# salesforce/gorp

Measured on AMD Instinct MI355X. Metric: lines/sec (Gorp.extract: product-DFA match + capture offsets; results as narrow rows (int8 id + uint8 offsets, 9 B/line)), higher is better.
Workload: dtype u8

## Files before the change

gorp_amd/csrc/gx_kernels.hip:

```cpp
#include "gx_rows.hpp"
#include "gx_hop_dev.hpp"

namespace gx {

namespace {

constexpr int GENERIC_MAX_REGS = 96;

template <typename CH>
__device__ __forceinline__ int class_of(const GxDev& T, CH ch) {
    uint32_t c = static_cast<uint32_t>(ch);
    if (sizeof(CH) == 1 || c < 256u) return T.cls256[c];
    int lo = 0, hi = T.n_hi;
    while (hi - lo > 1) {
        int mid = (lo + hi) >> 1;
        if (T.hi_lo[mid] <= c) lo = mid; else hi = mid;
    }
    return T.hi_cls[lo];
}

template <typename CH>
__device__ bool pike_capture(const GxDev& T, int k, const CH* __restrict__ s, int64_t len, int32_t* __restrict__ scratch, int32_t* __restrict__ caps_out) {
    const uint32_t base = T.pike_off[k], n_inst = T.pike_off[k + 1] - base;
    const uint32_t* code = T.pike_code + 2ull * base;
// ... 389 lines not shown
            const uint4 w0 = make_uint4(wv.x, wv.y, wv.z, wv.w);
            const bool full0 = rel + 16u <= len;
            const uint32_t bx = outside_bits(w0.x, lo4, k4), by = outside_bits(w0.y, lo4, k4);
            const uint32_t bz = outside_bits(w0.z, lo4, k4), bw = outside_bits(w0.w, lo4, k4);
            const bool ok0 = full0 & (((or3(bx, by, bz) | bw) & HI_BITS) == 0u);
            bool step = act && !ok0;
            uint32_t mask = 0xFFFFu;
            if (step && !full0) {
                mask = window_mask(0u, len, rel);
                step = !partial_window_ok(bx, by, bz, bw, mask);
            }
            const bool masked = __any(step && !full0);
            if (step) {
                if (want_caps) {
                    if (L.simple_ops) {
                        if (!masked) row = steps16<TIER, true, false, true>(w0, mask, W, row, rel, regs);
                        else row = steps16<TIER, true, true, true>(w0, mask, W, row, rel, regs);
                    } else {
                        if (!masked) row = steps16<TIER, true, false, false>(w0, mask, W, row, rel, regs);
                        else row = steps16<TIER, true, true, false>(w0, mask, W, row, rel, regs);
                    }
                } else {
                    if (!masked) row = steps16<TIER, false, false, false>(w0, mask, W, row, rel, regs);
                    else row = steps16<TIER, false, true, false>(w0, mask, W, row, rel, regs);
                }
                const uint32_t acc = state_acc<TIER>(W, row);
                lo4 = splat_byte0(acc);
                k4 = splat_byte1(acc);
            }
            more = more && row != dead_row;
        }
        if (walking) pos += SLICE_BYTES;
        __builtin_amdgcn_fence(__ATOMIC_RELEASE, "wavefront");
        __builtin_amdgcn_wave_barrier();
    }
}

template <typename OFF, int TIER>
hipError_t launch_slices_t(const GxDev& dev, const GxLds& lds, const uint8_t* lds_image, const uint8_t* at_global, dim3 grid, dim3 block,
                           const GxBatch& b, hipStream_t stream) {
    hipError_t e = allow_full_lds(&k_extract_slices<OFF, TIER>);
    if (e != hipSuccess) return e;
    hipLaunchKernelGGL((k_extract_slices<OFF, TIER>), grid, block, lds.total_bytes, stream, dev, lds, lds_image, at_global,
                       static_cast<const uint8_t*>(b.data), static_cast<const OFF*>(b.offsets), b.n, row_out(dev, b), b.match_only, b.strip_eol);
    return hipGetLastError();
}

#ifndef GX_HOP_LEAVE
#define GX_HOP_LEAVE 24u
#endif
#ifndef GX_HOP_SERVICE
#define GX_HOP_SERVICE 64u
#endif
constexpr uint64_t HOP_POOL_CHUNK = 64;
constexpr uint32_t HOP_SLICE = GX_HOP_SLICE_BYTES, HOP_SLICE_ROW = GX_HOP_SLICE_BYTES + 16u, HOP_SLICE_KEEP = 24;

typedef __attribute__((address_space(1))) const UnalignedWindow GlobalWindow;
template <bool WIDE, bool GUARDED>
__device__ __forceinline__ u32x4 load_chunk16(const uint8_t* src, const uint8_t* data_end, uint32_t units, uint32_t& high) {
    u32x4 a = {0u, 0u, 0u, 0u}, b2 = {0u, 0u, 0u, 0u};
    if (!GUARDED) {
        a = reinterpret_cast<GlobalWindow*>(reinterpret_cast<uintptr_t>(src))->v;
        if (WIDE) b2 = reinterpret_cast<GlobalWindow*>(reinterpret_cast<uintptr_t>(src + 16))->v;
    } else {
        uint32_t w[8] = {0, 0, 0, 0, 0, 0, 0, 0};
#pragma nounroll
        for (int q = 0; q < (WIDE ? 32 : 16); ++q)
            if (src + q < data_end) w[q >> 2] |= static_cast<uint32_t>(src[q]) << ((q & 3) * 8);
        a = u32x4{w[0], w[1], w[2], w[3]}; b2 = u32x4{w[4], w[5], w[6], w[7]};
    }
    if (!WIDE) return a;
    const uint32_t hi[8] = {a.x, a.y, a.z, a.w, b2.x, b2.y, b2.z, b2.w};
    uint32_t acc = 0u;
#pragma unroll
    for (uint32_t q = 0; q < 8u; ++q) {
        uint32_t m = 0xFF00FF00u;
        if (2u * q + 1u >= units) m = 2u * q >= units ? 0u : 0x0000FF00u;
        acc |= hi[q] & m;
    }
    high |= acc;
    return u32x4{__builtin_amdgcn_perm(a.y, a.x, 0x06040200u), __builtin_amdgcn_perm(a.w, a.z, 0x06040200u),
                 __builtin_amdgcn_perm(b2.y, b2.x, 0x06040200u), __builtin_amdgcn_perm(b2.w, b2.z, 0x06040200u)};
}
__device__ __forceinline__ bool chunk_in_run(const u32x4& v, uint32_t runinfo) {
    const uint32_t lo4 = splat_byte0(runinfo), k4 = splat_byte1(runinfo);
    const uint32_t f = (v.x | (v.x - lo4) | (v.x + k4)) | (v.y | (v.y - lo4) | (v.y + k4)) | (v.z | (v.z - lo4) | (v.z + k4)) | (v.w | (v.w - lo4) | (v.w + k4));
    return (f & HI_BITS) == 0u;
}
#ifndef GX_HOP_SPEC
#define GX_HOP_SPEC 1
#endif
#ifndef GX_HOP_SPEC_UNITS
#define GX_HOP_SPEC_UNITS 24
#endif
#ifndef GX_HOP_SPEC_BATCH
#define GX_HOP_SPEC_BATCH 8u
#endif
#ifndef GX_HOP_SPEC_MIN
#define GX_HOP_SPEC_MIN 0u
#endif


template <typename OFF, bool WIDE>
__global__ void __launch_bounds__(768) __attribute__((amdgpu_waves_per_eu(1, 3)))
k_extract_hop_slices(GxDev T, GxLds L, const uint8_t* __restrict__ lds_image, const uint8_t* __restrict__ at_global,
                     const uint8_t* __restrict__ data, const OFF* __restrict__ off, uint64_t n, RowOut out, int match_only, int strip_eol,
                     uint32_t* __restrict__ oversize_flag, uint32_t seq, unsigned long long* __restrict__ stamps,
                     uint32_t* __restrict__ pool_ctr, uint32_t pool_base, uint64_t n_static,
                     uint8_t* __restrict__ wide_flags, uint32_t* __restrict__ wide_any) {
    {
        extern __shared__ __attribute__((aligned(16))) uint8_t gx_smem[];
        const uint4* src = reinterpret_cast<const uint4*>(lds_image);
        uint4* dst = reinterpret_cast<uint4*>(gx_smem);
        for (uint32_t c = threadIdx.x; c < L.table_bytes / 16; c += blockDim.x) dst[c] = src[c];
    }
    __syncthreads();
#ifdef GX_DEV
    unsigned long long ph[6] = {0, 0, 0, 0, 0, 0}, ph_t = __builtin_amdgcn_s_memtime();
    unsigned long long dv[6] = {0, 0, 0, 0, 0, 0};
    const unsigned long long hs_begin = __builtin_amdgcn_s_memrealtime();
#define HS_STAMP(slot) do { const unsigned long long now_ = __builtin_amdgcn_s_memtime(); ph[slot] += now_ - ph_t; ph_t = now_; } while (0)
#else
#define HS_STAMP(slot) do { } while (0)
#endif
    HopTab H;
    H.rows = at_global;
    H.hops = at_global + L.c_base;
    H.row_bytes = L.row_bytes;
    H.info_off = L.ncls * 4u;
    H.n_hot = L.rec_indexed;
    H.lrow_cols = (2u * L.ncls + 3u) & ~3u;
    H.sets = L.hop_sets;
    const uint32_t lane = threadIdx.x & 63u;
    const uint32_t wave = threadIdx.x >> 6;
    const uint32_t slice = L.stage + wave * L.stage_bytes;
    const uint32_t regs = L.regs + wave * L.regs_wave_bytes + 128u + lane * 2u;
    const uint8_t* data_end = data + (static_cast<uint64_t>(off[n]) << (WIDE ? 1 : 0));
    const uint32_t row0 = match_only ? L.m_start : L.u_start, dead_row = match_only ? L.m_dead : L.u_dead;
    const uint8_t* fin_g = L.at != 0u ? nullptr : at_global + L.fin_tags;
    const uint32_t fin_lds = L.at;

    const uint64_t nwaves = static_cast<uint64_t>(gridDim.x) * L.nwaves;
    const uint64_t per_wave = (n_static + nwaves - 1) / nwaves;
    const uint64_t wid = static_cast<uint64_t>(blockIdx.x) * L.nwaves + wave;
    const uint64_t range_lo = min(n_static, wid * per_wave);
    uint64_t range_hi = min(n_static, range_lo + per_wave);
    uint64_t next = range_lo;
    const uint64_t pool_chunks = (n - n_static + HOP_POOL_CHUNK - 1) / HOP_POOL_CHUNK;
    bool pool_done = pool_ctr == nullptr;

    bool has_line = false;
    uint64_t i = 0, o0 = 0;
    uint32_t len = 0, pos = 0, row = row0;
    const uint32_t my = slice + lane * HOP_SLICE_ROW;
    bool line_wide = false;
    const uint64_t total_units = static_cast<uint64_t>(off[n]);
    uint64_t win_base = ~0ull;
    OFF w_lo = 0, w_hi = 0;
    auto refill = [&](uint64_t base) {
        win_base = base;
        const uint64_t a = min(base + lane, n);
        w_lo = off[a];
        w_hi = off[min(a + 1u, n)];
    };
    refill(range_lo);
    FinAhead F;
    bool fin_here = false;
    uint32_t near_end = 0u;
    HopKept K;
    const bool all_hot = L.rec_indexed >= L.sort_chunk;

    for (;;) {
        const bool finished = has_line && (pos >= len || row == dead_row);
        const uint32_t idle = static_cast<uint32_t>(__popcll(__ballot(finished || !has_line)));
        const bool service = idle >= GX_HOP_SERVICE || !__any(has_line && !finished);
        if (service && finished) {
            const bool rows_here = !(WIDE && line_wide);
            if (!match_only) lds_st<uint16_t>(regs - 128u, static_cast<uint16_t>(len));
            if (!match_only && L.fin_state_off != 0u) {
                const uint8_t* recp = at_global + L.fin_state_off + static_cast<uint64_t>(row) * L.fin_state_rec;
                if (!fin_here) F.load(recp, T.max_groups);
                if (rows_here) store_row<TIER_HOP>(out, i, 0, F.at(recp), regs, len, T.max_groups, L.fin_unset);
                fin_here = false;
            } else {
                const int32_t hot_info = static_cast<int16_t>(lds_ld<uint16_t>(L.acc_tab + 2u * min(row, H.n_hot - 1u)));
                int32_t info = hot_info >= 0 && !match_only ? hot_info * 16 : hot_info;
                if (row >= H.n_hot) info = *reinterpret_cast<const int32_t*>(H.rows + (static_cast<uint64_t>(row) * H.row_bytes + H.info_off));
                if (match_only) out.id(i, info);
                else if (rows_here) store_row<TIER_HOP>(out, i, info, fin_rec<TIER_HOP>(info, fin_lds, fin_g), regs, len, T.max_groups, L.fin_unset);
            }
            if (WIDE) {
                wide_flags[i] = line_wide ? 1 : 0;
                if (line_wide) __hip_atomic_store(wide_any, seq, __ATOMIC_RELAXED, __HIP_MEMORY_SCOPE_AGENT);
            }
            has_line = false;
        }
#ifdef GX_DEV
        if (service) ++dv[3];
#endif
        HS_STAMP(5);
        if (service && next >= range_hi && !pool_done) {
            uint32_t t = 0u;
            if (lane == 0u) t = __hip_atomic_fetch_add(pool_ctr, 1u, __ATOMIC_RELAXED, __HIP_MEMORY_SCOPE_AGENT) - pool_base;
            t = static_cast<uint32_t>(__builtin_amdgcn_readfirstlane(static_cast<int>(t)));
            if (t < pool_chunks) {
                next = n_static + static_cast<uint64_t>(t) * HOP_POOL_CHUNK;
                range_hi = min(n, next + HOP_POOL_CHUNK);
            } else pool_done = true;
        }
        const uint64_t free_mask = __ballot(!has_line);
        if (service && free_mask && next < range_hi) {
            const uint32_t rank = static_cast<uint32_t>(__popcll(free_mask & ((1ull << lane) - 1ull)));
            const uint64_t cand = next + rank;
            const uint32_t n_free = static_cast<uint32_t>(__popcll(free_mask));
            const bool in_win = next >= win_base && next - win_base + n_free <= 64u;
            OFF o_lo = 0, o_hi = 0;
            if (in_win) {
                const int src = static_cast<int>(static_cast<uint32_t>(next - win_base) + rank) & 63;
                o_lo = __shfl(w_lo, src);
                o_hi = __shfl(w_hi, src);
            }
            if (!has_line && cand < range_hi) {
                i = cand;
                if (!in_win) { o_lo = off[i]; o_hi = off[i + 1]; }
                o0 = o_lo;
                int64_t len64 = static_cast<int64_t>(static_cast<uint64_t>(o_hi) - o0);
                if (strip_eol) len64 = WIDE ? trim_eol(reinterpret_cast<const uint16_t*>(data) + o0, len64) : trim_eol(data + o0, len64);
                line_wide = false;
                if (WIDE && len64 > 65535) wide_flags[i] = 0;
                if (len64 > 65535) {
                    announce_left_line(oversize_flag, seq);
                } else {
                    has_line = true;
                    len = static_cast<uint32_t>(len64);
                    pos = 0;
                    row = row0;
                    near_end = static_cast<uint64_t>(o_hi) + 16u > total_units ? 0x10000u : 0u;
                }
            }
            next = min(range_hi, next + static_cast<uint64_t>(n_free));
            refill(next);
// ... 157 lines not shown
                    }
                }
                __builtin_amdgcn_fence(__ATOMIC_RELEASE, "wavefront");
                __builtin_amdgcn_wave_barrier();
                __builtin_amdgcn_fence(__ATOMIC_ACQUIRE, "wavefront");
                uint32_t got = 0u;
                bool alive = longrun;
                for (uint32_t k = 0; __builtin_amdgcn_ballot_w64(alive && k < units) != 0ull; ++k) {
                    const bool look = alive && k < units;
                    const uint32_t bits = look ? lds_ld<uint8_t>(BITS + first + k) : 0xFFu;
                    if (look) {
                        got += 16u * static_cast<uint32_t>(__builtin_ctz(~bits | 0x100u));
                        alive = bits == 0xFFu;
                    }
                }
                extra = min(got, rest0);
            }
        }
        pos += extra;
        if (!match_only && L.fin_state_off != 0u) {
            if (has_line && !fin_here && (pos >= len || row == dead_row)) {
                F.load(at_global + L.fin_state_off + static_cast<uint64_t>(row) * L.fin_state_rec, T.max_groups);
                fin_here = true;
            }
        }
        __builtin_amdgcn_fence(__ATOMIC_RELEASE, "wavefront");
        __builtin_amdgcn_wave_barrier();
        HS_STAMP(2);
#ifdef GX_DEV
        ++ph[4];
#endif
    }
#ifdef GX_DEV
    if (stamps && lane == 0) {
        unsigned long long* st = stamps + 16ull * (static_cast<uint64_t>(blockIdx.x) * L.nwaves + wave);
        for (int q = 0; q < 6; ++q) st[q] = ph[q];
        st[6] = hs_begin;
        st[7] = __builtin_amdgcn_s_memrealtime();
        for (int q = 0; q < 4; ++q) st[8 + q] = dv[q];
        st[12] = K.dev_iters;
        st[13] = K.dev_lane_iters;
    }
#endif
}

}

namespace {
uint64_t hop_slices_blocks(uint64_t n, uint32_t nwaves, int num_cus) {
    uint64_t blocks = static_cast<uint64_t>(num_cus);
    const uint64_t need = (n + 256ull * nwaves - 1) / (256ull * nwaves);
    return blocks > need ? need : blocks;
}
uint64_t hop_slices_static(uint64_t n) { return n - (n / 4) / HOP_POOL_CHUNK * HOP_POOL_CHUNK; }
}

uint32_t hop_slices_tickets(uint64_t n, uint32_t nwaves, int num_cus) {
    if (n == 0) return 0u;
    const uint64_t chunks = (n - hop_slices_static(n) + HOP_POOL_CHUNK - 1) / HOP_POOL_CHUNK;
    return static_cast<uint32_t>(chunks + hop_slices_blocks(n, nwaves, num_cus) * nwaves);
}

hipError_t launch_extract_hop_slices(const GxDev& dev, const GxLds& lds, const uint8_t* lds_image, const uint8_t* at_global, int num_cus,
                                     const GxBatch& b, hipStream_t stream, unsigned long long* stamps) {
    if (b.n == 0) return hipSuccess;
    const uint64_t blocks = hop_slices_blocks(b.n, lds.nwaves, num_cus);
    const uint64_t n_static = b.chunk_ctr ? hop_slices_static(b.n) : b.n;
    const dim3 grid(static_cast<unsigned>(blocks)), block(lds.nwaves * 64);
    auto go = [&](auto kernel, auto offsets) -> hipError_t {
        hipError_t e = allow_full_lds(kernel);
        if (e != hipSuccess) return e;
        hipLaunchKernelGGL(kernel, grid, block, lds.total_bytes, stream, dev, lds, lds_image, at_global, static_cast<const uint8_t*>(b.data), offsets, b.n, row_out(dev, b),
                           (b.match_only != 0 || !dev.has_capture) ? 1 : 0, b.strip_eol, b.oversize_flag, b.seq, stamps, b.chunk_ctr, b.chunk_base, n_static,
                           b.wide_flags, b.wide_any);
        return hipGetLastError();
    };
    if (b.wide) {
        if (!b.wide_flags || !b.wide_any) return hipErrorInvalidValue;
        if (b.offsets64) return go(&k_extract_hop_slices<uint64_t, true>, static_cast<const uint64_t*>(b.offsets));
        return go(&k_extract_hop_slices<uint32_t, true>, static_cast<const uint32_t*>(b.offsets));
    }
    if (b.offsets64) return go(&k_extract_hop_slices<uint64_t, false>, static_cast<const uint64_t*>(b.offsets));
    return go(&k_extract_hop_slices<uint32_t, false>, static_cast<const uint32_t*>(b.offsets));
}

hipError_t launch_narrow_units(const GxBatch& b, uint8_t* bytes_at_first_unit, uint8_t* flags, hipStream_t stream) {
    if (b.n == 0) return hipSuccess;
    hipError_t e = hipMemsetAsync(flags, 0, b.n, stream);
    if (e != hipSuccess) return e;
    const dim3 grid(256u * 16u), block(256);
    if (b.offsets64) hipLaunchKernelGGL((k_narrow_units<uint64_t>), grid, block, 0, stream, static_cast<const uint16_t*>(b.data), static_cast<const uint64_t*>(b.offsets), b.n, bytes_at_first_unit, flags);
    else hipLaunchKernelGGL((k_narrow_units<uint32_t>), grid, block, 0, stream, static_cast<const uint16_t*>(b.data), static_cast<const uint32_t*>(b.offsets), b.n, bytes_at_first_unit, flags);
    return hipGetLastError();
}
hipError_t launch_extract_flagged(const GxDev& dev, const GxBatch& b, const uint8_t* flags, hipStream_t stream, const uint32_t* any_word) {
    if (b.n == 0) return hipSuccess;
    const dim3 grid(dev.pike_off ? dev.pike_blocks : 256u * 4u), block(256);
    const uint16_t* units = static_cast<const uint16_t*>(b.data);
#define GX_FLAGGED(OFF, MS, NEXT) hipLaunchKernelGGL((k_extract_flagged<OFF, MS>), grid, block, 0, stream, dev, units, static_cast<const OFF*>(b.offsets), b.n, flags, row_out(dev, b), b.match_only, NEXT, b.strip_eol, any_word, b.seq)
    if (b.offsets64) { if (dev.m_next16) GX_FLAGGED(uint64_t, uint16_t, dev.m_next16); else GX_FLAGGED(uint64_t, uint32_t, dev.m_next32); }
    else { if (dev.m_next16) GX_FLAGGED(uint32_t, uint16_t, dev.m_next16); else GX_FLAGGED(uint32_t, uint32_t, dev.m_next32); }
#undef GX_FLAGGED
    return hipGetLastError();
}
hipError_t launch_extract_listed(const GxDev& dev, const GxBatch& b, const uint64_t* list, uint64_t count, hipStream_t stream) {
    if (count == 0) return hipSuccess;
    if (!b.wide || !b.offsets64) return hipErrorInvalidValue;
// ... 61 lines not shown
```

gorp_amd/csrc/gx_lanes.hip:

```cpp
#include "gx_rows.hpp"

namespace gx {

namespace {

struct LanesIO {
    const uint8_t* image;
    const uint8_t* at_global;
    const uint8_t* data;
    const void* off;
    uint64_t n;
    RowOut rows;
    uint32_t* oversize_flag;
    uint32_t seq;
    int32_t max_groups;
    int32_t strip_eol;
    uint32_t chunk_lines;
    uint32_t sort_lds;
    uint32_t* chunk_ctr;
    uint32_t chunk_base;
#ifdef GX_DEV
    unsigned long long* stamps;
#endif
};
// ... 121 lines not shown
            bool more = valid && !oversize && len > 0u;
            auto line_chunk = [&](uint32_t at_byte, bool wanted) -> u32x4 {
                u32x4 v = {0u, 0u, 0u, 0u};
                if (wanted && at_byte < len) {
                    const uint8_t* src = line + at_byte;
                    if (src + 16 <= data_end) v = reinterpret_cast<const UnalignedWindow*>(src)->v;
                    else {
                        uint32_t w[4] = {0, 0, 0, 0};
                        for (int b = 0; b < 16; ++b)
                            if (src + b < data_end) w[b >> 2] |= static_cast<uint32_t>(src[b]) << ((b & 3) * 8);
                        v = u32x4{w[0], w[1], w[2], w[3]};
                    }
                }
                return v;
            };
            for (uint32_t seg = 0; __any(more); seg += KCH * 16u) {
                u32x4 pre[KCH];
    #pragma unroll
                for (int k = 0; k < KCH; ++k) pre[k] = line_chunk(seg + 16u * k, more);
    #pragma unroll 1
                for (int k = 0; k < KCH; ++k) {
                    const uint32_t rel = seg + 16u * k;
                    const bool act = more && rel < len;
                    if (!__any(act)) break;
                    const uint4 w0 = make_uint4(pre[0].x, pre[0].y, pre[0].z, pre[0].w);
    #pragma unroll
                    for (int q = 0; q + 1 < KCH; ++q) pre[q] = pre[q + 1];
                    const bool full0 = rel + 16u <= len;
                    const uint32_t bx = outside_bits(w0.x, lo4, k4), by = outside_bits(w0.y, lo4, k4);
                    const uint32_t bz = outside_bits(w0.z, lo4, k4), bw = outside_bits(w0.w, lo4, k4);
                    const bool ok0 = full0 & (((or3(bx, by, bz) | bw) & HI_BITS) == 0u);
                    bool step = act && !ok0;
                    uint32_t mask = 0xFFFFu;
                    if (step && !full0) {
                        mask = window_mask(0u, len, rel);
                        step = !partial_window_ok(bx, by, bz, bw, mask);
                    }
                    const bool masked = __any(step && !full0);
                    if (step) {
                        if (!masked) row = steps16<TIER, CAPTURE, false, SIMPLE>(w0, mask, W, row, rel, regs);
                        else row = steps16<TIER, CAPTURE, true, SIMPLE>(w0, mask, W, row, rel, regs);
                        acc = state_acc<TIER>(W, row);
                        lo4 = splat_byte0(acc);
                        k4 = splat_byte1(acc);
                    }
                    more = more && row != dead_row && rel + 16u < len;
                }
            }

            const int32_t info = state_info<TIER>(W, row);
            if (!CAPTURE) {
                if (valid && !oversize) io.rows.match_id[i] = info;
            } else {
                auto result = [&](auto emit) { return line_result<TIER>(info, L.fin_tags, fin_g, regs, len, G, emit); };
                const bool full_tile = contiguous && __all(valid) && !__any(oversize);
                const uint32_t area_bytes = L.regs_wave_bytes - L.stage_bytes;
                if (!PACKED) store_tile<ROWS_DENSE, false>(io.rows, slots, i, lane, valid && !oversize, false, out_area, area_bytes, len, result);
                else if (io.rows.format == ROWS_U8) store_tile<ROWS_U8, true>(io.rows, slots, i, lane, valid && !oversize, full_tile, out_area, area_bytes, len, result);
                else store_tile<ROWS_U16, false>(io.rows, slots, i, lane, valid && !oversize, full_tile, out_area, area_bytes, len, result);
            }
            __builtin_amdgcn_fence(__ATOMIC_ACQ_REL, "wavefront");
            __builtin_amdgcn_wave_barrier();
            if (!SORTED) j = next_ticket();
        }
        if (!SORTED) break;
        __syncthreads();
    }
#ifdef GX_DEV
    if (io.stamps && threadIdx.x == 0) {
        io.stamps[2 * blockIdx.x] = __builtin_amdgcn_s_memtime() - dev_t0;
        io.stamps[2 * blockIdx.x + 1] = __builtin_amdgcn_s_memrealtime() - dev_r0;
    }
#endif
}

template <typename OFF, int TIER, bool CAPTURE, bool SIMPLE, bool PACKED, bool SORTED>
hipError_t launch_lanes_s(const GxLds& lds, const LanesIO& io, dim3 grid, hipStream_t stream) {
    constexpr int KCH = 13;
    hipError_t e = allow_full_lds(&k_extract_lanes<OFF, KCH, TIER, CAPTURE, SIMPLE, PACKED, SORTED>);
    if (e != hipSuccess) return e;
    hipLaunchKernelGGL((k_extract_lanes<OFF, KCH, TIER, CAPTURE, SIMPLE, PACKED, SORTED>), grid, dim3(lds.nwaves * 64), lds.total_bytes, stream, lds, io);
    return hipGetLastError();
}
template <typename OFF, int TIER, bool CAPTURE, bool SIMPLE, bool PACKED>
hipError_t launch_lanes_t(const GxLds& lds, const LanesIO& io, dim3 grid, hipStream_t stream) {
    if (io.chunk_lines) return launch_lanes_s<OFF, TIER, CAPTURE, SIMPLE, PACKED, true>(lds, io, grid, stream);
    return launch_lanes_s<OFF, TIER, CAPTURE, SIMPLE, PACKED, false>(lds, io, grid, stream);
}
template <typename OFF, int TIER>
hipError_t launch_lanes_m(bool capture, bool simple, bool packed, const GxLds& lds, const LanesIO& io, dim3 grid, hipStream_t stream) {
    if (!capture) return launch_lanes_t<OFF, TIER, false, false, false>(lds, io, grid, stream);
    if (simple) return packed ? launch_lanes_t<OFF, TIER, true, true, true>(lds, io, grid, stream) : launch_lanes_t<OFF, TIER, true, true, false>(lds, io, grid, stream);
    return packed ? launch_lanes_t<OFF, TIER, true, false, true>(lds, io, grid, stream) : launch_lanes_t<OFF, TIER, true, false, false>(lds, io, grid, stream);
}

}

uint32_t lanes_sorted_tickets(uint64_t n, uint32_t chunk_lines, int num_cus) {
    const uint64_t nchunks = (n + chunk_lines - 1) / chunk_lines;
    return static_cast<uint32_t>(nchunks + (static_cast<uint64_t>(num_cus) < nchunks ? static_cast<uint64_t>(num_cus) : nchunks));
}

hipError_t launch_extract_lanes(const GxDev& dev, const GxLds& lds, const uint8_t* lds_image, const uint8_t* at_global, int num_cus,
                                const GxBatch& b, hipStream_t stream, unsigned long long* dev_stamps) {
    if (b.n == 0) return hipSuccess;
    const uint64_t tiles = (b.n + 63) >> 6;
    uint64_t blocks = static_cast<uint64_t>(num_cus);
// ... 47 lines not shown
```

gorp_amd/csrc/gx_rows.hpp:

```cpp
#pragma once
#include "gx_walk.hpp"

namespace gx {

struct RowOut {
    int32_t* match_id;
    int32_t* caps;
    uint8_t* rows;
    unsigned long long* overflow;
    RowFormat format;
    uint32_t slots;

    __device__ __forceinline__ void id(uint64_t i, int32_t k) const {
        if (format == ROWS_U8) rows[i * row_bytes(ROWS_U8, slots)] = static_cast<uint8_t>(encode_id(ROWS_U8, k));
        else if (format == ROWS_U16) *reinterpret_cast<uint16_t*>(rows + i * row_bytes(ROWS_U16, slots)) = static_cast<uint16_t>(encode_id(ROWS_U16, k));
        else match_id[i] = k;
    }
    __device__ __forceinline__ void cap(uint64_t i, int t, int32_t v) const {
        if (format == ROWS_DENSE) { caps[i * static_cast<uint64_t>(slots) + t] = v; return; }
        const RowUnit u = encode_offset(format, v);
        if (u.clipped && overflow) atomicAdd(overflow, 1ull);
        uint8_t* p = rows + i * row_bytes(format, slots) + row_unit_bytes(format) * (1u + t);
        if (format == ROWS_U8) *p = static_cast<uint8_t>(u.unit);
        else *reinterpret_cast<uint16_t*>(p) = static_cast<uint16_t>(u.unit);
// ... 29 lines not shown
    }
}
template <int TIER>
__device__ __forceinline__ void resolve_tags(const u32x4& t, uint32_t regs, uint32_t len, uint32_t hop_unset, int32_t (&pb)[4], int32_t (&pe)[4]) {
    uint32_t tw[4], vb[4], ve[4];
    tag_columns<TIER>(t, regs, tw, vb, ve);
#pragma unroll
    for (int q = 0; q < 4; ++q) tag_offsets<TIER>(tw[q], vb[q], ve[q], len, hop_unset, pb[q], pe[q]);
}

struct FinRec {
    uint32_t fin_lds;
    const uint8_t* fin_g;
    uint32_t rec;
    bool global;
    __device__ __forceinline__ u32x4 tags(int g0) const {
        return global ? *reinterpret_cast<const u32x4*>(fin_g + rec + 4u * g0) : lds_ld<u32x4>(fin_lds + rec + 4u * g0);
    }
    __device__ __forceinline__ uint32_t id_of(int G) const {
        const uint32_t id_at = rec + 16u * static_cast<uint32_t>((G + 3) >> 2);
        return global ? *reinterpret_cast<const uint16_t*>(fin_g + id_at) : lds_ld<uint16_t>(fin_lds + id_at);
    }
};
template <int TIER>
__device__ __forceinline__ FinRec fin_rec(int32_t info, uint32_t fin_lds, const uint8_t* fin_g) {
    const bool global = TIER == TIER_L2 || TIER == TIER_RECG || (TIER == TIER_HOP && fin_g != nullptr);
    return FinRec{fin_lds, fin_g, info >= 0 ? static_cast<uint32_t>(info) : 0u, global};
}

struct FinAhead {
    u32x4 t0 = {0u, 0u, 0u, 0u}, t1 = {0u, 0u, 0u, 0u}, t2 = {0u, 0u, 0u, 0u};
    uint32_t id = 0u;
    __device__ __forceinline__ void load(const uint8_t* __restrict__ recp, int G) {
        const int nblk = (G + 3) >> 2;
        t0 = *reinterpret_cast<const u32x4*>(recp);
        t1 = *reinterpret_cast<const u32x4*>(recp + (nblk > 1 ? 16 : 0));
        t2 = *reinterpret_cast<const u32x4*>(recp + (nblk > 2 ? 32 : 0));
        id = *reinterpret_cast<const uint16_t*>(recp + 16 * nblk);
    }
    struct At {
        u32x4 t0, t1, t2;
        uint32_t id;
        const uint8_t* recp;
        __device__ __forceinline__ u32x4 tags(int g0) const {
            if (g0 >= 12) return *reinterpret_cast<const u32x4*>(recp + 4 * g0);
            const u32x4 a = t0, b = t1, c = t2;
            return g0 == 0 ? a : g0 == 4 ? b : c;
        }
        __device__ __forceinline__ uint32_t id_of(int) const { return id; }
    };
    __device__ __forceinline__ At at(const uint8_t* recp) const { return At{t0, t1, t2, id, recp}; }
};

template <int TIER, typename EMIT>
__device__ __forceinline__ int32_t line_result(int32_t info, uint32_t fin_lds, const uint8_t* fin_g, uint32_t regs, uint32_t len, int G,
                                               EMIT emit, uint32_t hop_unset = 0u) {
    const uint32_t rec = info >= 0 ? static_cast<uint32_t>(info) : 0u;
    const uint32_t id_at = rec + 16u * static_cast<uint32_t>((G + 3) >> 2);
    uint32_t id;
    const bool FIN_GLOBAL = TIER == TIER_L2 || TIER == TIER_RECG || (TIER == TIER_HOP && fin_g != nullptr);
    if (FIN_GLOBAL) id = *reinterpret_cast<const uint16_t*>(fin_g + id_at);
    else id = lds_ld<uint16_t>(fin_lds + id_at);
    for (int g0 = 0; g0 < G; g0 += 4) {
        u32x4 t;
        if (FIN_GLOBAL) t = *reinterpret_cast<const u32x4*>(fin_g + rec + 4u * g0);
        else t = lds_ld<u32x4>(fin_lds + rec + 4u * g0);
        uint32_t tw[4], vb[4], ve[4];
        tag_columns<TIER>(t, regs, tw, vb, ve);
#pragma unroll
        for (int q = 0; q < 4; ++q) {
            if (g0 + q < G) {
                int32_t pb, pe;
                tag_offsets<TIER>(tw[q], vb[q], ve[q], len, hop_unset, pb, pe);
                emit(g0 + q, pb, pe);
            }
        }
    }
    return info >= 0 ? static_cast<int32_t>(static_cast<int16_t>(id)) : info;
}

struct __attribute__((packed)) UnalignedU32x4 { u32x4 v; };
struct __attribute__((packed)) UnalignedU32x2 { u32x2 v; };
struct __attribute__((packed)) UnalignedU32 { uint32_t v; };
struct __attribute__((packed)) UnalignedU16 { uint16_t v; };

template <int TIER, typename REC>
__device__ __forceinline__ void store_row(const RowOut& out, uint64_t i, int32_t info, const REC& rec, uint32_t regs, uint32_t len, int G,
                                          uint32_t hop_unset = 0u) {
    const RowFormat f = out.format;
    const int32_t mid = info >= 0 ? static_cast<int32_t>(static_cast<int16_t>(rec.id_of(G))) : info;
    uint8_t* row = f != ROWS_DENSE ? out.rows + i * row_bytes(f, out.slots) : reinterpret_cast<uint8_t*>(out.caps + i * static_cast<uint64_t>(out.slots));
    if (f == ROWS_DENSE) out.match_id[i] = mid;
    uint32_t carry = encode_id(f, mid);
    uint32_t clipped = 0u;
    const bool may_clip = __builtin_amdgcn_ballot_w64(len > static_cast<uint32_t>(row_max_offset(f))) != 0ull;
    for (int g0 = 0; g0 < G; g0 += 4) {
        int32_t pb[4], pe[4];
        resolve_tags<TIER>(rec.tags(g0), regs, len, hop_unset, pb, pe);
        const int cnt = G - g0 < 4 ? G - g0 : 4;
        if (f == ROWS_DENSE) {
            uint8_t* dst = row + 8u * g0;
            if (cnt == 4) {
                reinterpret_cast<UnalignedU32x4*>(dst)->v = u32x4{static_cast<uint32_t>(pb[0]), static_cast<uint32_t>(pe[0]), static_cast<uint32_t>(pb[1]), static_cast<uint32_t>(pe[1])};
                reinterpret_cast<UnalignedU32x4*>(dst + 16)->v = u32x4{static_cast<uint32_t>(pb[2]), static_cast<uint32_t>(pe[2]), static_cast<uint32_t>(pb[3]), static_cast<uint32_t>(pe[3])};
            } else {
#pragma unroll
                for (int q = 0; q < 4; ++q) if (q < cnt) reinterpret_cast<UnalignedU32x2*>(dst + 8 * q)->v = u32x2{static_cast<uint32_t>(pb[q]), static_cast<uint32_t>(pe[q])};
            }
            continue;
        }
        uint32_t hb[4], he[4];
        if (!may_clip) {
#pragma unroll
            for (int q = 0; q < 4; ++q) { hb[q] = static_cast<uint32_t>(pb[q]) & row_unset(f); he[q] = static_cast<uint32_t>(pe[q]) & row_unset(f); }
        } else {
#pragma unroll
            for (int q = 0; q < 4; ++q) {
                const RowUnit b = encode_offset(f, pb[q]), e = encode_offset(f, pe[q]);
                hb[q] = b.unit;
                he[q] = e.unit;
                clipped += b.clipped + e.clipped;
            }
        }
        if (f == ROWS_U16) {
            uint8_t* dst = row + 4u * g0;
            if (cnt == 4) {
                reinterpret_cast<UnalignedU32x4*>(dst)->v = u32x4{carry | hb[0] << 16, he[0] | hb[1] << 16, he[1] | hb[2] << 16, he[2] | hb[3] << 16};
                carry = he[3];
            } else {
#pragma unroll
                for (int q = 0; q < 4; ++q) {
                    if (q >= cnt) break;
                    reinterpret_cast<UnalignedU32*>(dst + 4 * q)->v = carry | hb[q] << 16;
                    carry = he[q];
                }
            }
        } else {
            uint8_t* dst = row + 2u * g0;
            if (cnt == 4) {
                reinterpret_cast<UnalignedU32x2*>(dst)->v = u32x2{carry | hb[0] << 8 | he[0] << 16 | hb[1] << 24, he[1] | hb[2] << 8 | he[2] << 16 | hb[3] << 24};
                carry = he[3];
            } else {
#pragma unroll
                for (int q = 0; q < 4; ++q) {
                    if (q >= cnt) break;
                    reinterpret_cast<UnalignedU16*>(dst + 2 * q)->v = static_cast<uint16_t>(carry | hb[q] << 8);
                    carry = he[q];
                }
            }
        }
    }
    if (f != ROWS_DENSE) {
        if (f == ROWS_U8) row[2 * G] = static_cast<uint8_t>(carry);
        else reinterpret_cast<UnalignedU16*>(row + 4 * G)->v = static_cast<uint16_t>(carry);
        if (clipped && out.overflow) atomicAdd(out.overflow, static_cast<unsigned long long>(clipped));
    }
}

template <RowFormat F, bool CLIP, typename RESULT>
__device__ __forceinline__ void store_tile(const RowOut& out, uint32_t slots, uint64_t i, uint32_t lane, bool valid, bool full, uint32_t area,
                                           uint32_t area_bytes, uint32_t len, RESULT result, uint32_t dev_flags = 0u) {
    (void)dev_flags;
    if (F != ROWS_DENSE) {
        constexpr uint32_t U = row_unit_bytes(F);
        const uint32_t row_b = row_bytes(F, slots);
        constexpr int32_t max = row_max_offset(F);
        auto st = [&](uint32_t lds_at, int32_t v) {
            if (U == 1) lds_st<uint8_t>(lds_at, static_cast<uint8_t>(v));
            else lds_st<uint16_t>(lds_at, static_cast<uint16_t>(v));
        };
        const bool rows_aligned = (reinterpret_cast<uintptr_t>(out.rows) & 15u) == 0u;
        uint32_t clipped = 0;
        if (full && rows_aligned && 64u * row_b + 16u <= area_bytes) {
            const uint32_t my_row = area + lane * row_b;
            int32_t id;
            if (!CLIP || !__any(len > static_cast<uint32_t>(max))) {
                id = result([&](int g, int32_t pb, int32_t pe) {
                    st(my_row + U + 2u * U * g, pb);
                    st(my_row + 2u * U + 2u * U * g, pe);
                });
            } else {
                id = result([&](int g, int32_t pb, int32_t pe) {
                    clipped += (pb > max ? 1u : 0u) + (pe > max ? 1u : 0u);
                    st(my_row + U + 2u * U * g, pb > max ? max : pb);
                    st(my_row + 2u * U + 2u * U * g, pe > max ? max : pe);
                });
            }
            st(my_row, id);
            __builtin_amdgcn_fence(__ATOMIC_ACQ_REL, "wavefront");
            __builtin_amdgcn_wave_barrier();
            uint8_t* out_rows = out.rows + (i - lane) * static_cast<uint64_t>(row_b);
            for (uint32_t c = lane; c < 4u * row_b; c += 64u) {
#ifdef GX_DEV
                if (dev_flags & 2u) { __builtin_nontemporal_store(lds_ld<u32x4>(area + (c << 4)), reinterpret_cast<u32x4*>(out_rows + (c << 4))); continue; }
                if ((dev_flags & 4u) && c != 0u) continue;
#endif
                *reinterpret_cast<u32x4*>(out_rows + (c << 4)) = lds_ld<u32x4>(area + (c << 4));
            }
        } else if (valid) {
            using Unit = typename std::conditional<U == 1, uint8_t, uint16_t>::type;
            Unit* rp = reinterpret_cast<Unit*>(out.rows) + i * static_cast<uint64_t>(1u + slots);
            auto gst = [&](uint32_t k, int32_t v) { rp[k] = static_cast<Unit>(v); };
            const int32_t id = result([&](int g, int32_t pb, int32_t pe) {
                if (CLIP) {
                    clipped += (pb > max ? 1u : 0u) + (pe > max ? 1u : 0u);
                    gst(1 + 2 * g, pb > max ? max : pb);
                    gst(2 + 2 * g, pe > max ? max : pe);
                } else {
                    gst(1 + 2 * g, pb);
                    gst(2 + 2 * g, pe);
                }
            });
            gst(0, id);
        }
        if (CLIP && out.overflow && __any(clipped != 0u)) {
            uint32_t sum = clipped;
#pragma unroll
            for (int d = 32; d >= 1; d >>= 1) sum += static_cast<uint32_t>(__shfl_xor(static_cast<int>(sum), d));
            if (lane == 0) atomicAdd(out.overflow, static_cast<unsigned long long>(sum));
        }
    } else {
        const uint32_t row_b = slots * 4u;
        const bool caps_aligned = ((reinterpret_cast<uintptr_t>(out.caps) | reinterpret_cast<uintptr_t>(out.match_id)) & 15u) == 0u;
        if (full && caps_aligned && 64u * row_b + 256u <= area_bytes) {
            const uint32_t my_row = area + lane * row_b;
            const int32_t id = result([&](int g, int32_t pb, int32_t pe) {
                lds_st<u32x2>(my_row + 8u * g, u32x2{static_cast<uint32_t>(pb), static_cast<uint32_t>(pe)});
            });
            const uint32_t ids = area + 64u * row_b;
            lds_st<uint32_t>(ids + 4u * lane, static_cast<uint32_t>(id));
            __builtin_amdgcn_fence(__ATOMIC_ACQ_REL, "wavefront");
            __builtin_amdgcn_wave_barrier();
            uint8_t* dst = reinterpret_cast<uint8_t*>(out.caps + (i - lane) * static_cast<uint64_t>(slots));
            for (uint32_t c = lane; c < 4u * row_b; c += 64u)
                *reinterpret_cast<u32x4*>(dst + (c << 4)) = lds_ld<u32x4>(area + (c << 4));
            if (lane < 16u)
                *reinterpret_cast<u32x4*>(out.match_id + (i - lane) + 4u * lane) = lds_ld<u32x4>(ids + 16u * lane);
        } else if (valid) {
            int32_t* cp = out.caps + i * static_cast<uint64_t>(slots);
            out.match_id[i] = result([&](int g, int32_t pb, int32_t pe) {
                cp[2 * g] = pb;
                cp[2 * g + 1] = pe;
            });
        }
    }
}

}
```

gorp_amd/csrc/gx_service.hip:

```cpp
#include "gx_tile_body.hpp"

namespace gx {

namespace {

__device__ __forceinline__ uint32_t sys_load(const uint32_t* p) { return __hip_atomic_load(p, __ATOMIC_RELAXED, __HIP_MEMORY_SCOPE_SYSTEM); }

template <int MODE>
__global__ void __launch_bounds__(64)
k_one_service(GxLds L, const uint8_t* __restrict__ image, const uint32_t* __restrict__ mailbox, int32_t* __restrict__ answer, uint32_t* __restrict__ state,
              uint32_t last, int max_groups, unsigned long long idle_ticks, unsigned long long life_ticks) {
    {
        extern __shared__ __attribute__((aligned(16))) uint8_t gx_smem[];
        const uint4* src = reinterpret_cast<const uint4*>(image);
        uint4* dst = reinterpret_cast<uint4*>(gx_smem);
        for (uint32_t c = threadIdx.x; c < L.table_bytes / 16; c += blockDim.x) dst[c] = src[c];
    }
    __syncthreads();
    const uint32_t lane = threadIdx.x;
    WalkTab W;
    W.at = nullptr;
    W.row_bytes = L.row_bytes;
    W.ops_off = L.ops_off;
    W.ops = L.ops;
    W.acc_tab = L.acc_tab;
    W.ncls = L.ncls;
    W.indexed = L.rec_indexed;
    const uint32_t stage = L.stage;
    const uint32_t regs = L.regs + 128u + lane * 2u;
    const int G = max_groups;
    const unsigned long long born = __builtin_amdgcn_s_memrealtime();
    unsigned long long idle_since = born;
    bool announced = false;
    for (;;) {
        uint32_t w = lane < 16u ? sys_load(mailbox + lane) : 0u;
        const uint32_t seq = static_cast<uint32_t>(__builtin_amdgcn_readlane(static_cast<int>(w), 0));
        const uint32_t head = static_cast<uint32_t>(__builtin_amdgcn_readlane(static_cast<int>(w), 1));
        if (seq != last) {
            const uint32_t len = head & 0xFFFFu;
            if (announced) { if (lane == 0) __hip_atomic_store(state, 1u, __ATOMIC_RELAXED, __HIP_MEMORY_SCOPE_SYSTEM); announced = false; }
            if (lane >= 2u && lane < 16u) lds_st<uint32_t>(stage + 4u * (lane - 2u), w);
            if (len > 56u) {
                const uint32_t lines = (len - 56u + 59u) / 60u;
                for (uint32_t c0 = 0; c0 < lines; c0 += 4u) {
                    const uint32_t cl = c0 + (lane >> 4), d = lane & 15u;
                    const bool mine = cl < lines;
                    for (;;) {
                        const uint32_t v = mine ? sys_load(mailbox + 16u * (1u + cl) + d) : seq;
                        const bool tag_ok = d != 0u || v == seq;
                        if (__builtin_amdgcn_ballot_w64(!tag_ok) == 0ull) {
                            if (mine && d != 0u) lds_st<uint32_t>(stage + 56u + 60u * cl + 4u * (d - 1u), v);
                            break;
                        }
                        __builtin_amdgcn_s_sleep(2);
                    }
                }
            }
            __builtin_amdgcn_fence(__ATOMIC_RELEASE, "wavefront");
            __builtin_amdgcn_wave_barrier();
            __builtin_amdgcn_fence(__ATOMIC_ACQUIRE, "wavefront");
            const bool on = lane == 0u;
            const uint32_t out = stage + L.stage_bytes - 272u;
            int32_t result;
            if (MODE == 0) {
                const uint32_t mrow = walk<TIER_LDS, false, false>(W, stage, 0u, false, L.m_start, 0u, on ? len : 0u, on, L.m_dead, regs);
                result = state_info<TIER_LDS>(W, mrow);
                if (on) lds_st<uint32_t>(out, static_cast<uint32_t>(result));
            } else {
                const uint32_t urow = walk<TIER_LDS, true, true>(W, stage, 0u, false, L.u_start, 0u, on ? len : 0u, on, L.u_dead, regs);
                const int32_t info = state_info<TIER_LDS>(W, urow);
                result = line_result<TIER_LDS>(info, L.fin_tags, nullptr, regs, len, G, [&](int g, int32_t pb, int32_t pe) {
                    if (on) lds_st<u32x2>(out + 4u + 8u * g, u32x2{static_cast<uint32_t>(pb), static_cast<uint32_t>(pe)});
                });
                if (on) lds_st<uint32_t>(out, static_cast<uint32_t>(result));
            }
            __builtin_amdgcn_fence(__ATOMIC_RELEASE, "wavefront");
            __builtin_amdgcn_wave_barrier();
            __builtin_amdgcn_fence(__ATOMIC_ACQUIRE, "wavefront");
            if (lane < 1u + 2u * static_cast<uint32_t>(MODE == 0 ? 0 : G)) answer[lane] = static_cast<int32_t>(lds_ld<uint32_t>(out + 4u * lane));
            __builtin_amdgcn_fence(__ATOMIC_RELEASE, "");
            if (on) __hip_atomic_store(reinterpret_cast<uint32_t*>(answer) + 1 + 2 * max_groups, seq, __ATOMIC_RELEASE, __HIP_MEMORY_SCOPE_SYSTEM);
            last = seq;
            idle_since = __builtin_amdgcn_s_memrealtime();
            if (idle_since - born > life_ticks) {
                if (lane == 0) __hip_atomic_store(state, 2u, __ATOMIC_RELEASE, __HIP_MEMORY_SCOPE_SYSTEM);
                announced = true;
                continue;
            }
            continue;
        }
        if (announced) break;
        const unsigned long long now = __builtin_amdgcn_s_memrealtime();
        if ((head >> 16) & 1u || now - idle_since > idle_ticks || now - born > life_ticks) {
            if (lane == 0) __hip_atomic_store(state, 2u, __ATOMIC_RELEASE, __HIP_MEMORY_SCOPE_SYSTEM);
            __builtin_amdgcn_fence(__ATOMIC_SEQ_CST, "");
            announced = true;
            continue;
        }
        __builtin_amdgcn_s_sleep(1);
    }
}

}

hipError_t launch_one_service(int mode, const GxLds& lds, const uint8_t* lds_image, const uint32_t* mailbox, int32_t* answer, uint32_t* state,
                              uint32_t last_seq, int max_groups, unsigned long long idle_ticks, unsigned long long life_ticks, hipStream_t stream) {
    if (mode == 0) {
        hipError_t e = allow_full_lds(&k_one_service<0>);
        if (e != hipSuccess) return e;
        hipLaunchKernelGGL((k_one_service<0>), dim3(1), dim3(64), lds.total_bytes, stream, lds, lds_image, mailbox, answer, state, last_seq, max_groups, idle_ticks, life_ticks);
    } else {
        hipError_t e = allow_full_lds(&k_one_service<1>);
        if (e != hipSuccess) return e;
        hipLaunchKernelGGL((k_one_service<1>), dim3(1), dim3(64), lds.total_bytes, stream, lds, lds_image, mailbox, answer, state, last_seq, max_groups, idle_ticks, life_ticks);
    }
    return hipGetLastError();
}

}
```

gorp_amd/csrc/gx_tile_body.hpp:

```cpp
#pragma once
#include "gx_rows.hpp"
#include "gx_hop_dev.hpp"

namespace gx {

namespace {

struct TileIO {
    const uint8_t* image;
    const uint8_t* at_global;
    const uint8_t* data;
    const void* off;
    uint64_t n;
    RowOut rows;
    uint32_t* oversize_flag;
    uint32_t seq;
    int32_t max_groups;
    int32_t strip_eol;
    uint32_t* steal;
    uint32_t steal_parity;
    uint32_t share64;
    uint8_t* wide_flags;
    uint32_t* wide_any;
    int32_t* state_out;
// ... 401 lines not shown
        if (io.strip_eol && cur.mode != 2) {
            if (end > start && lds_ld<uint8_t>(stage + end - 1u) == 0x0Au) --end;
            if (end > start && lds_ld<uint8_t>(stage + end - 1u) == 0x0Du) --end;
        }
        if (cur.mode == 2) {
            if (lane == cur.a) announce_left_line(io.oversize_flag, io.seq);
        } else if (MODE == 0 && HOP) {
            const uint32_t mrow = walk_hop<false>(H, L.rec_indexed >= L.sort_chunk, stage, L.m_start, start, end, true, L.m_dead, regs, hop_second);
            int32_t first = static_cast<int16_t>(lds_ld<uint16_t>(L.acc_tab + 2u * min(mrow, H.n_hot - 1u)));
            if (wave_any(mrow >= H.n_hot)) {
                if (mrow >= H.n_hot) first = *reinterpret_cast<const int32_t*>(H.rows + (static_cast<uint64_t>(mrow) * H.row_bytes + H.info_off));
            }
            if (valid) io.rows.match_id[i] = first;
            GX_STAMP(2);
        } else if (MODE == 0) {
            const uint32_t mrow = walk<TIER, false, false>(Wm, stage, bitmap, use_map, L.m_start, start, end, true, L.m_dead, regs);
            if (valid) io.rows.match_id[i] = state_info<TIER>(Wm, mrow);
            if ((TIER == TIER_LDS || TIER == TIER_L2) && io.state_out && valid)
                io.state_out[i] = mrow == L.m_dead ? -1 : static_cast<int32_t>(TIER == TIER_LDS ? (mrow - L.m_start) / L.row_bytes : mrow - L.m_start);
            GX_STAMP(2);
        } else {
            int32_t info;
            if (HOP) {
                const uint32_t urow = walk_hop<true>(H, L.rec_indexed >= L.sort_chunk, stage, L.u_start, start, end, true, L.u_dead, regs, hop_second);
                const int32_t hot_info = static_cast<int16_t>(lds_ld<uint16_t>(L.acc_tab + 2u * min(urow, H.n_hot - 1u)));
                info = hot_info >= 0 ? hot_info * 16 : hot_info;
                if (wave_any(urow >= H.n_hot)) {
                    if (urow >= H.n_hot) info = *reinterpret_cast<const int32_t*>(H.rows + (static_cast<uint64_t>(urow) * H.row_bytes + H.info_off));
                }
            } else if (MODE == 1 || L.u_start != 0xFFFFFFFFu) {
                uint32_t urow;
                if (MODE == 1 || L.simple_ops) urow = walk<TIER, true, true>(Wc, stage, bitmap, use_map, L.u_start, start, end, true, L.u_dead, regs);
                else urow = walk<TIER, true, false>(Wc, stage, bitmap, use_map, L.u_start, start, end, true, L.u_dead, regs);
                info = state_info<TIER>(Wc, urow);
            } else {
                const uint32_t mrow = walk<TIER, false, false>(Wm, stage, bitmap, use_map, L.m_start, start, end, true, L.m_dead, regs);
                const int32_t k = state_info<TIER>(Wm, mrow);
                info = k;
                uint32_t crow = GT ? 0u : L.m_dead;
                if (k >= 0) crow = lds_ld<uint32_t>(L.c_rule + 8u * k);
                if (L.simple_ops) crow = walk<TIER, true, true>(Wc, stage, bitmap, use_map, crow, start, end, k >= 0, 0xFFFFFFFFu, regs);
                else crow = walk<TIER, true, false>(Wc, stage, bitmap, use_map, crow, start, end, k >= 0, 0xFFFFFFFFu, regs);
                if (k >= 0) {
                    info = state_info<TIER>(Wc, crow);
                    if (info < 0) info = -2 - k;
                }
            }
            GX_STAMP(2);
            if (WIDE && wide_line) info = -1;
            const uint32_t len = end - start;
            if (HOP) lds_st<uint16_t>(regs - 128u, static_cast<uint16_t>(len));
            const uint8_t* fin_g = GT && !(HOP && L.at != 0u) ? io.at_global + L.fin_tags : nullptr;
            const uint32_t fin_lds = HOP ? L.at : L.fin_tags;
            auto result = [&](auto emit) { return line_result<TIER>(info, fin_lds, fin_g, regs, len, G, emit, L.fin_unset); };
            const bool full_tile = cur.a == 0u && cur.b == 64u;
#ifdef GX_DEV
            const uint32_t dev_flags = io.dev_flags;
#else
            const uint32_t dev_flags = 0u;
#endif
            constexpr RowFormat FMT = PACKED == 2 ? ROWS_U8 : PACKED == 1 ? ROWS_U16 : ROWS_DENSE;
            store_tile<FMT, FMT == ROWS_U8>(io.rows, slots, i, lane, valid, full_tile, stage, L.stage_bytes, len, result, dev_flags);
        }
        if (WIDE) {
            if (valid || (cur.mode == 2 && lane == cur.a)) io.wide_flags[i] = (wide_line && cur.mode != 2) ? 1 : 0;
            if (__builtin_amdgcn_ballot_w64(wide_line && valid && cur.mode != 2) != 0ull && lane == 0)
                __hip_atomic_store(io.wide_any, io.seq, __ATOMIC_RELAXED, __HIP_MEMORY_SCOPE_AGENT);
        }
        __builtin_amdgcn_fence(__ATOMIC_ACQ_REL, "wavefront");
        __builtin_amdgcn_wave_barrier();
        GX_STAMP(3);
#ifdef GX_DEV
        ++dev_tiles;
#endif
        if (!has_next) break;
        if (!same_group) {
            t1 = t2;
            need_t2 = true;
        }
        cur = nxt;
        tile = ntile;
        no0 = nno0;
        no1 = nno1;
    }
#ifdef GX_DEV
    if (io.stamps && lane == 0) {
        unsigned long long* s = io.stamps + 8ull * (static_cast<uint64_t>(blockIdx.x) * L.nwaves + wave);
        for (int q = 0; q < 4; ++q) s[q] = phase_cycles[q];
        s[4] = dev_begin;
        s[5] = __builtin_amdgcn_s_memrealtime();
        s[6] = dev_tiles;
        uint32_t xcc;
        asm volatile("s_getreg_b32 %0, hwreg(HW_REG_XCC_ID)" : "=s"(xcc));
        s[7] = xcc;
    }
#endif
}

template <typename OFF, int KCH, int TIER, int MODE, int PACKED, bool WIDE = false>
hipError_t launch_tile_p(const GxLds& lds, const TileIO& io, dim3 grid, dim3 block, hipStream_t stream) {
    hipError_t e = allow_full_lds(&k_extract_tile<OFF, KCH, TIER, MODE, PACKED, WIDE>);
    if (e != hipSuccess) return e;
    hipLaunchKernelGGL((k_extract_tile<OFF, KCH, TIER, MODE, PACKED, WIDE>), grid, block, lds.total_bytes, stream, lds, io);
    return hipGetLastError();
}
template <typename OFF, int KCH, int TIER, int MODE, bool WIDE = false>
hipError_t launch_tile_t(const GxLds& lds, const TileIO& io, dim3 grid, dim3 block, hipStream_t stream) {
// ... 40 lines not shown
```

Before: 27.83 billion.

## Stage full-wave hop rows through LDS for coalesced 16-byte stores

In the hop-slices kernel, when a service step finds all 64 lanes finishing consecutive lines with aligned output, rows are staged in LDS and written with coalesced 16-byte stores instead of per-lane scattered row stores. Static per-wave ranges and the static/pool split are rounded to 64-line multiples so tiles line up with wave lanes. line_result is refactored to take a record accessor (fin_rec / F.at), and callers are updated. This adds ballot/readfirstlane checks on every service step, and the condition may rarely hold because lanes finish lines at different times.

```diff
diff --git a/gorp_amd/csrc/gx_kernels.hip b/gorp_amd/csrc/gx_kernels.hip
--- a/gorp_amd/csrc/gx_kernels.hip
+++ b/gorp_amd/csrc/gx_kernels.hip
@@ -465,6 +465,10 @@
 #ifndef GX_HOP_SERVICE
 #define GX_HOP_SERVICE 64u
 #endif
+#ifndef GX_HOP_ROW_BLOCK
+#define GX_HOP_ROW_BLOCK 1
+#endif
+constexpr uint64_t HOP_RANGE_ALIGN = 64;
 constexpr uint64_t HOP_POOL_CHUNK = 64;
 constexpr uint32_t HOP_SLICE = GX_HOP_SLICE_BYTES, HOP_SLICE_ROW = GX_HOP_SLICE_BYTES + 16u, HOP_SLICE_KEEP = 24;
 
@@ -513,6 +517,15 @@
 #define GX_HOP_SPEC_MIN 0u
 #endif
 
+
+template <typename RESULT>
+__device__ __forceinline__ void store_gen(const RowOut& out, uint64_t i, uint32_t lane, uint32_t area, uint32_t area_bytes, uint32_t len, RESULT result) {
+    if (out.format == ROWS_DENSE) store_tile<ROWS_DENSE, false, true>(out, out.slots, i, lane, true, true, area, area_bytes, len, result);
+    else if (out.format == ROWS_U8) store_tile<ROWS_U8, true, true>(out, out.slots, i, lane, true, true, area, area_bytes, len, result);
+    else store_tile<ROWS_U16, true, true>(out, out.slots, i, lane, true, true, area, area_bytes, len, result);
+    __builtin_amdgcn_fence(__ATOMIC_RELEASE, "wavefront");
+    __builtin_amdgcn_wave_barrier();
+}
 
 template <typename OFF, bool WIDE>
 __global__ void __launch_bounds__(768) __attribute__((amdgpu_waves_per_eu(1, 3)))
@@ -554,7 +567,7 @@
     const uint32_t fin_lds = L.at;
 
     const uint64_t nwaves = static_cast<uint64_t>(gridDim.x) * L.nwaves;
-    const uint64_t per_wave = (n_static + nwaves - 1) / nwaves;
+    const uint64_t per_wave = ((n_static + nwaves - 1) / nwaves + HOP_RANGE_ALIGN - 1) / HOP_RANGE_ALIGN * HOP_RANGE_ALIGN;
     const uint64_t wid = static_cast<uint64_t>(blockIdx.x) * L.nwaves + wave;
     const uint64_t range_lo = min(n_static, wid * per_wave);
     uint64_t range_hi = min(n_static, range_lo + per_wave);
@@ -587,19 +600,33 @@
         const bool finished = has_line && (pos >= len || row == dead_row);
         const uint32_t idle = static_cast<uint32_t>(__popcll(__ballot(finished || !has_line)));
         const bool service = idle >= GX_HOP_SERVICE || !__any(has_line && !finished);
+
+        bool gen_full = false;
+        if (GX_HOP_ROW_BLOCK && service && !match_only) {
+            const uint64_t i0 = static_cast<uint64_t>(static_cast<uint32_t>(__builtin_amdgcn_readfirstlane(static_cast<int>(i >> 32)))) << 32 |
+                                static_cast<uint32_t>(__builtin_amdgcn_readfirstlane(static_cast<int>(i)));
+            bool room;
+            if (out.format == ROWS_DENSE) room = ((reinterpret_cast<uintptr_t>(out.caps) | reinterpret_cast<uintptr_t>(out.match_id) | (i0 << 2)) & 15u) == 0u &&
+                                                 64u * 4u * out.slots + 256u <= L.stage_bytes;
+            else room = ((reinterpret_cast<uintptr_t>(out.rows) | i0 * row_bytes(out.format, out.slots)) & 15u) == 0u &&
+                        64u * row_bytes(out.format, out.slots) + 16u <= L.stage_bytes;
+            gen_full = room && __builtin_amdgcn_ballot_w64(finished && i == i0 + lane && !(WIDE && line_wide)) == ~0ull;
+        }
         if (service && finished) {
             const bool rows_here = !(WIDE && line_wide);
             if (!match_only) lds_st<uint16_t>(regs - 128u, static_cast<uint16_t>(len));
             if (!match_only && L.fin_state_off != 0u) {
                 const uint8_t* recp = at_global + L.fin_state_off + static_cast<uint64_t>(row) * L.fin_state_rec;
                 if (!fin_here) F.load(recp, T.max_groups);
-                if (rows_here) store_row<TIER_HOP>(out, i, 0, F.at(recp), regs, len, T.max_groups, L.fin_unset);
+                if (gen_full) store_gen(out, i, lane, slice, L.stage_bytes, len, [&](auto emit) { return line_result<TIER_HOP>(0, F.at(recp), regs, len, T.max_groups, emit, L.fin_unset); });
+                else if (rows_here) store_row<TIER_HOP>(out, i, 0, F.at(recp), regs, len, T.max_groups, L.fin_unset);
                 fin_here = false;
             } else {
                 const int32_t hot_info = static_cast<int16_t>(lds_ld<uint16_t>(L.acc_tab + 2u * min(row, H.n_hot - 1u)));
                 int32_t info = hot_info >= 0 && !match_only ? hot_info * 16 : hot_info;
                 if (row >= H.n_hot) info = *reinterpret_cast<const int32_t*>(H.rows + (static_cast<uint64_t>(row) * H.row_bytes + H.info_off));
                 if (match_only) out.id(i, info);
+                else if (gen_full) store_gen(out, i, lane, slice, L.stage_bytes, len, [&](auto emit) { return line_result<TIER_HOP>(info, fin_rec<TIER_HOP>(info, fin_lds, fin_g), regs, len, T.max_groups, emit, L.fin_unset); });
                 else if (rows_here) store_row<TIER_HOP>(out, i, info, fin_rec<TIER_HOP>(info, fin_lds, fin_g), regs, len, T.max_groups, L.fin_unset);
             }
             if (WIDE) {
@@ -863,7 +890,7 @@
     const uint64_t need = (n + 256ull * nwaves - 1) / (256ull * nwaves);
     return blocks > need ? need : blocks;
 }
-uint64_t hop_slices_static(uint64_t n) { return n - (n / 4) / HOP_POOL_CHUNK * HOP_POOL_CHUNK; }
+uint64_t hop_slices_static(uint64_t n) { return (n - (n / 4) / HOP_POOL_CHUNK * HOP_POOL_CHUNK) / HOP_RANGE_ALIGN * HOP_RANGE_ALIGN; }
 }
 
 uint32_t hop_slices_tickets(uint64_t n, uint32_t nwaves, int num_cus) {
diff --git a/gorp_amd/csrc/gx_lanes.hip b/gorp_amd/csrc/gx_lanes.hip
--- a/gorp_amd/csrc/gx_lanes.hip
+++ b/gorp_amd/csrc/gx_lanes.hip
@@ -197,7 +197,7 @@
             if (!CAPTURE) {
                 if (valid && !oversize) io.rows.match_id[i] = info;
             } else {
-                auto result = [&](auto emit) { return line_result<TIER>(info, L.fin_tags, fin_g, regs, len, G, emit); };
+                auto result = [&](auto emit) { return line_result<TIER>(info, fin_rec<TIER>(info, L.fin_tags, fin_g), regs, len, G, emit); };
                 const bool full_tile = contiguous && __all(valid) && !__any(oversize);
                 const uint32_t area_bytes = L.regs_wave_bytes - L.stage_bytes;
                 if (!PACKED) store_tile<ROWS_DENSE, false>(io.rows, slots, i, lane, valid && !oversize, false, out_area, area_bytes, len, result);
diff --git a/gorp_amd/csrc/gx_rows.hpp b/gorp_amd/csrc/gx_rows.hpp
--- a/gorp_amd/csrc/gx_rows.hpp
+++ b/gorp_amd/csrc/gx_rows.hpp
@@ -105,21 +105,12 @@
     __device__ __forceinline__ At at(const uint8_t* recp) const { return At{t0, t1, t2, id, recp}; }
 };
 
-template <int TIER, typename EMIT>
-__device__ __forceinline__ int32_t line_result(int32_t info, uint32_t fin_lds, const uint8_t* fin_g, uint32_t regs, uint32_t len, int G,
-                                               EMIT emit, uint32_t hop_unset = 0u) {
-    const uint32_t rec = info >= 0 ? static_cast<uint32_t>(info) : 0u;
-    const uint32_t id_at = rec + 16u * static_cast<uint32_t>((G + 3) >> 2);
-    uint32_t id;
-    const bool FIN_GLOBAL = TIER == TIER_L2 || TIER == TIER_RECG || (TIER == TIER_HOP && fin_g != nullptr);
-    if (FIN_GLOBAL) id = *reinterpret_cast<const uint16_t*>(fin_g + id_at);
-    else id = lds_ld<uint16_t>(fin_lds + id_at);
+template <int TIER, typename REC, typename EMIT>
+__device__ __forceinline__ int32_t line_result(int32_t info, const REC& rec, uint32_t regs, uint32_t len, int G, EMIT emit, uint32_t hop_unset = 0u) {
+    const uint32_t id = rec.id_of(G);
     for (int g0 = 0; g0 < G; g0 += 4) {
-        u32x4 t;
-        if (FIN_GLOBAL) t = *reinterpret_cast<const u32x4*>(fin_g + rec + 4u * g0);
-        else t = lds_ld<u32x4>(fin_lds + rec + 4u * g0);
         uint32_t tw[4], vb[4], ve[4];
-        tag_columns<TIER>(t, regs, tw, vb, ve);
+        tag_columns<TIER>(rec.tags(g0), regs, tw, vb, ve);
 #pragma unroll
         for (int q = 0; q < 4; ++q) {
             if (g0 + q < G) {
@@ -210,7 +201,7 @@
     }
 }
 
-template <RowFormat F, bool CLIP, typename RESULT>
+template <RowFormat F, bool CLIP, bool FULL_ONLY = false, typename RESULT>
 __device__ __forceinline__ void store_tile(const RowOut& out, uint32_t slots, uint64_t i, uint32_t lane, bool valid, bool full, uint32_t area,
                                            uint32_t area_bytes, uint32_t len, RESULT result, uint32_t dev_flags = 0u) {
     (void)dev_flags;
@@ -250,7 +241,7 @@
 #endif
                 *reinterpret_cast<u32x4*>(out_rows + (c << 4)) = lds_ld<u32x4>(area + (c << 4));
             }
-        } else if (valid) {
+        } else if (!FULL_ONLY && valid) {
             using Unit = typename std::conditional<U == 1, uint8_t, uint16_t>::type;
             Unit* rp = reinterpret_cast<Unit*>(out.rows) + i * static_cast<uint64_t>(1u + slots);
             auto gst = [&](uint32_t k, int32_t v) { rp[k] = static_cast<Unit>(v); };
@@ -289,7 +280,7 @@
                 *reinterpret_cast<u32x4*>(dst + (c << 4)) = lds_ld<u32x4>(area + (c << 4));
             if (lane < 16u)
                 *reinterpret_cast<u32x4*>(out.match_id + (i - lane) + 4u * lane) = lds_ld<u32x4>(ids + 16u * lane);
-        } else if (valid) {
+        } else if (!FULL_ONLY && valid) {
             int32_t* cp = out.caps + i * static_cast<uint64_t>(slots);
             out.match_id[i] = result([&](int g, int32_t pb, int32_t pe) {
                 cp[2 * g] = pb;
diff --git a/gorp_amd/csrc/gx_service.hip b/gorp_amd/csrc/gx_service.hip
--- a/gorp_amd/csrc/gx_service.hip
+++ b/gorp_amd/csrc/gx_service.hip
@@ -69,7 +69,7 @@
             } else {
                 const uint32_t urow = walk<TIER_LDS, true, true>(W, stage, 0u, false, L.u_start, 0u, on ? len : 0u, on, L.u_dead, regs);
                 const int32_t info = state_info<TIER_LDS>(W, urow);
-                result = line_result<TIER_LDS>(info, L.fin_tags, nullptr, regs, len, G, [&](int g, int32_t pb, int32_t pe) {
+                result = line_result<TIER_LDS>(info, fin_rec<TIER_LDS>(info, L.fin_tags, nullptr), regs, len, G, [&](int g, int32_t pb, int32_t pe) {
                     if (on) lds_st<u32x2>(out + 4u + 8u * g, u32x2{static_cast<uint32_t>(pb), static_cast<uint32_t>(pe)});
                 });
                 if (on) lds_st<uint32_t>(out, static_cast<uint32_t>(result));
diff --git a/gorp_amd/csrc/gx_tile_body.hpp b/gorp_amd/csrc/gx_tile_body.hpp
--- a/gorp_amd/csrc/gx_tile_body.hpp
+++ b/gorp_amd/csrc/gx_tile_body.hpp
@@ -477,7 +477,7 @@
             if (HOP) lds_st<uint16_t>(regs - 128u, static_cast<uint16_t>(len));
             const uint8_t* fin_g = GT && !(HOP && L.at != 0u) ? io.at_global + L.fin_tags : nullptr;
             const uint32_t fin_lds = HOP ? L.at : L.fin_tags;
-            auto result = [&](auto emit) { return line_result<TIER>(info, fin_lds, fin_g, regs, len, G, emit, L.fin_unset); };
+            auto result = [&](auto emit) { return line_result<TIER>(info, fin_rec<TIER>(info, fin_lds, fin_g), regs, len, G, emit, L.fin_unset); };
             const bool full_tile = cur.a == 0u && cur.b == 64u;
 #ifdef GX_DEV
             const uint32_t dev_flags = io.dev_flags;
```

New measurement: 27.81 billion. No clear change (-0.1%).
